# zafarrafii/Zaf-Python

Hardware: AMD Instinct MI355X
Metric: audio Msamples/sec (STFT win=2048 hop=1024) (higher is better)
Workload: dtype f32

## Files before the change

### zaf-python_amd/csrc/zafx_capi.cpp

```cpp
#include <dlfcn.h>

#include <algorithm>
#include <cmath>
#include <complex>
#include <cstdlib>
#include <cstring>
#include <map>
#include <mutex>
#include <string>
#include <utility>

#include "zafx_internal.hpp"

#ifndef ZAFX_STFT_FAT8_TABLES
#define ZAFX_STFT_FAT8_TABLES 0
#endif

namespace zafx {

static thread_local std::string g_err;
void set_error(const std::string& msg) { g_err = msg; }

hipError_t ensure_dynamic_lds(const void* kernel, int device, size_t bytes) {
    static std::mutex mu;
// ... 949 lines not shown
                    }
                    return cf32{(float)(scale * c), (float)(scale * sn)};
                };
                aux[(size_t)n] = root(2 * n * b2 + 2 * n * n, sin_);
                aux[(size_t)(N + n)] = root(2 * n * a2 + a2 * b2 + 2 * n * n + (sine ? 6 * D : 0), sout / L);
            }
            pl->kernel_name = "k_dct_bs32";
        } else {
            return bail("dct / dst: lengths above 8192 need N / 2 (types 2-4), N - 1 (dct type 1) or N + 1 (dst type 1) to be a power of two (at most 8192)");
        }
    } else {
        return bail("unknown plan kind");
    }
    pl->log2e = default_log2e(pl->log2nf);

    hipError_t e = hipSetDevice(device);
    if (e == hipSuccess) e = hipDeviceGetAttribute(&pl->n_cus, hipDeviceAttributeMultiprocessorCount, device);
    if (e == hipSuccess) e = hipStreamCreateWithFlags(&pl->stream, hipStreamNonBlocking);
    if (e == hipSuccess) e = hipEventCreate(&pl->ev0);
    if (e == hipSuccess) e = hipEventCreate(&pl->ev1);
    if (e == hipSuccess) {
        auto tw = is_cqt_family(kind) ? build_two_level_twiddles(pl->log2nf) : build_pass_twiddles(pl->log2nf, pl->log2e);
        if (is_cqt_family(kind) && cqt_split(pl->log2nf)) {
            const auto sub = build_pass_twiddles(10, 4);
            tw.insert(tw.end(), sub.begin(), sub.end());
        }
        if (tw.empty()) tw.push_back(cf32{1.f, 0.f});
        e = upload(&pl->d_tw_pass, tw.data(), tw.size() * sizeof(cf32));
        if (e == hipSuccess && (kind == ZAFX_STFT || kind == ZAFX_MEL || kind == ZAFX_MFCC) && (pl->log2nf == 10 || (ZAFX_STFT_FAT8_TABLES && pl->log2nf == 11 && kind == ZAFX_STFT))) {
            auto tw5 = build_pass_twiddles(pl->log2nf, 5);
            e = upload(&pl->d_tw_r32, tw5.data(), tw5.size() * sizeof(cf32));
        }
    }
    if (e == hipSuccess && (kind == ZAFX_STFT || kind == ZAFX_ISTFT || kind == ZAFX_MEL || kind == ZAFX_MFCC) && pl->log2nf == 11 && pl->prm.precision == ZAFX_PRECISION_F32) {
        const auto sub = build_pass_twiddles(10, 4);
        e = upload(&pl->d_tw_sub, sub.data(), sub.size() * sizeof(cf32));
    }
    if (e == hipSuccess && (kind == ZAFX_STFT || kind == ZAFX_ISTFT || kind == ZAFX_MEL || kind == ZAFX_MFCC) && pl->log2nf == 12 && pl->prm.precision == ZAFX_PRECISION_F32 && pl->bs_log2m == 0) {
        const auto sub = build_pass_twiddles(10, 4);
        e = upload(&pl->d_tw_sub, sub.data(), sub.size() * sizeof(cf32));
        std::vector<cf32> q(4096);
        for (int n = 0; n < 4096; ++n) q[(size_t)n] = unit_root(n, 8192);
        if (e == hipSuccess) e = upload(&pl->d_tw_quad, q.data(), q.size() * sizeof(cf32));
    }
    if (e == hipSuccess && kind == ZAFX_MDCT && pl->log2nf == 11 && pl->prm.precision == ZAFX_PRECISION_F32 && pl->bs_log2m == 0) {
        const auto sub = build_pass_twiddles(9, 3);
        e = upload(&pl->d_tw_sub, sub.data(), sub.size() * sizeof(cf32));
        std::vector<cf32> q(2048);
        for (int n = 0; n < 2048; ++n) q[(size_t)n] = unit_root(n, 2048);
        if (e == hipSuccess) e = upload(&pl->d_tw_quad, q.data(), q.size() * sizeof(cf32));
    }
    if (e == hipSuccess && kind == ZAFX_IMDCT && pl->log2nf == 11 && pl->prm.precision == ZAFX_PRECISION_F32 && pl->bs_log2m == 0) {
        const auto sub = build_pass_twiddles(10, 4);
        e = upload(&pl->d_tw_sub, sub.data(), sub.size() * sizeof(cf32));
        std::vector<cf32> q(2048);
        for (int n = 0; n < 2048; ++n) q[(size_t)n] = unit_root(n, 2048);
        if (e == hipSuccess) e = upload(&pl->d_tw_quad, q.data(), q.size() * sizeof(cf32));
    }
    if (e == hipSuccess && kind == ZAFX_MDCT && pl->log2nf == 10 && pl->prm.precision == ZAFX_PRECISION_F32 && pl->bs_log2m == 0) {
        const auto sub = build_pass_twiddles(9, 3);
        e = upload(&pl->d_tw_sub, sub.data(), sub.size() * sizeof(cf32));
        const int nf = pl->W / 4;
        std::vector<cf32> bt((size_t)nf + nf / 2);
        for (int s = 0; s < 2; ++s)
            for (int q = 0; q < nf / 2; ++q) bt[(size_t)s * (nf / 2) + q] = unit_root(8LL * (2 * q + s) + 1, 8LL * pl->W);
        for (int n = 0; n < nf / 2; ++n) bt[(size_t)nf + n] = unit_root(40LL * n + 1, 32LL * nf);
// ... 55 lines not shown
        } else if (cqt) {
            for (int k = 0; k < pl->W; ++k) tws[(size_t)k] = root(k, pl->W);
        } else {
            for (int k = 0; k <= n / 2; ++k) tws[(size_t)k] = root(k, pl->W);
        }
        if (e == hipSuccess) e = upload(&pl->d_tw64, tw.data(), tw.size() * sizeof(double2));
        if (e == hipSuccess) e = upload(&pl->d_tws64, tws.data(), tws.size() * sizeof(double2));
        pl->kernel_name = kind == ZAFX_STFT ? stft_f64_kernel_name() : kind == ZAFX_ISTFT ? istft_f64_kernel_name()
                          : kind == ZAFX_MDCT ? mdct_f64_kernel_name() : kind == ZAFX_IMDCT ? imdct_f64_kernel_name()
                          : cqt ? cqt_f64_kernel_name() : mel_f64_kernel_name();
        if (pl->bs_log2m > 0)
            pl->kernel_name = kind == ZAFX_ISTFT ? "k_ifft_frames_bs_f64" : kind == ZAFX_MDCT ? "k_mdct_bs_f64"
                              : kind == ZAFX_IMDCT ? "k_imdct_frames_bs_f64" : "k_stft_bs_f64";
    }
    if (e != hipSuccess) {
        zafx_plan_destroy(pl);
        return fail("zafx_plan_create", e);
    }
    *out = pl;
    return 0;
}

int zafx_plan_destroy(zafx_plan* pl) {
    if (!pl) return 0;
    (void)hipSetDevice(pl->device);
    if (pl->stream) (void)hipStreamSynchronize(pl->stream);
    for (int l = 0; l < 2; ++l)
        if (pl->lane_pcm[l]) (void)hipFree(pl->lane_pcm[l]);
    if (pl->d_window) (void)hipFree(pl->d_window);
    if (pl->d_matrix) (void)hipFree(pl->d_matrix);
    if (pl->d_wfold) (void)hipFree(pl->d_wfold);
    if (pl->d_tw_pass) (void)hipFree(pl->d_tw_pass);
    if (pl->d_tw_r32) (void)hipFree(pl->d_tw_r32);
    if (pl->d_tw_quad) (void)hipFree(pl->d_tw_quad);
    if (pl->d_tw_sub) (void)hipFree(pl->d_tw_sub);
    if (pl->d_tw_band) (void)hipFree(pl->d_tw_band);
    if (pl->d_fbw) (void)hipFree(pl->d_fbw);
    if (pl->d_fbw_meta) (void)hipFree(pl->d_fbw_meta);
    if (pl->d_dctw) (void)hipFree(pl->d_dctw);
    if (pl->d_tw_aux) (void)hipFree(pl->d_tw_aux);
    if (pl->d_indptr) (void)hipFree(pl->d_indptr);
    if (pl->d_indices) (void)hipFree(pl->d_indices);
    if (pl->d_values) (void)hipFree(pl->d_values);
    if (pl->d_cqt_waves) (void)hipFree(pl->d_cqt_waves);
    if (pl->d_cqt_addrs) (void)hipFree(pl->d_cqt_addrs);
    if (pl->d_cqt_vals) (void)hipFree(pl->d_cqt_vals);
    if (pl->d_cqt_mm_vals) (void)hipFree(pl->d_cqt_mm_vals);
    if (pl->d_cqt_mm_addr) (void)hipFree(pl->d_cqt_mm_addr);
    if (pl->d_cqt_mm_fin) (void)hipFree(pl->d_cqt_mm_fin);
    if (pl->d_window64) (void)hipFree(pl->d_window64);
    if (pl->d_tw64) (void)hipFree(pl->d_tw64);
    if (pl->d_tws64) (void)hipFree(pl->d_tws64);
    if (pl->d_scratch64) (void)hipFree(pl->d_scratch64);
    if (pl->d_fb64) (void)hipFree(pl->d_fb64);
    if (pl->d_fb64_meta) (void)hipFree(pl->d_fb64_meta);
    if (pl->d_dct64) (void)hipFree(pl->d_dct64);
    if (pl->d_cqt64_tw1) (void)hipFree(pl->d_cqt64_tw1);
    if (pl->d_cqt64_split) (void)hipFree(pl->d_cqt64_split);
    if (pl->d_cqt64_vals) (void)hipFree(pl->d_cqt64_vals);
    if (pl->d_cqt64_meta) (void)hipFree(pl->d_cqt64_meta);
    if (pl->d_cqt64_fin) (void)hipFree(pl->d_cqt64_fin);
    if (pl->d_mel64_stream) (void)hipFree(pl->d_mel64_stream);
    if (pl->d_mel64_fin) (void)hipFree(pl->d_mel64_fin);
    if (pl->d_mel64_dctT) (void)hipFree(pl->d_mel64_dctT);
    if (pl->d_values64) (void)hipFree(pl->d_values64);
    if (pl->d_bhat64) (void)hipFree(pl->d_bhat64);
// ... 838 lines not shown
```

### zaf-python_amd/csrc/zafx_fft.hpp

```cpp
#pragma once

#if defined(ZAFX_HOST_EMU)
#include <cmath>
struct float2 { float x, y; };
static inline float2 make_float2(float x, float y) { float2 r; r.x = x; r.y = y; return r; }
#define ZAFX_HD inline
#else
#include <hip/hip_runtime.h>

#include <type_traits>
#define ZAFX_HD __host__ __device__ __forceinline__
#endif

namespace zafx {

#if defined(__HIP_DEVICE_COMPILE__)
typedef float zafx_v2f __attribute__((ext_vector_type(2)));
__device__ __forceinline__ zafx_v2f to_v2(float2 a) { return __builtin_bit_cast(zafx_v2f, a); }
__device__ __forceinline__ float2 to_f2(zafx_v2f a) { return __builtin_bit_cast(float2, a); }
#define ZAFX_PK 1
#endif
#if defined(ZAFX_PK)
ZAFX_HD float2 cadd(float2 a, float2 b) { return to_f2(to_v2(a) + to_v2(b)); }
ZAFX_HD float2 csub(float2 a, float2 b) { return to_f2(to_v2(a) - to_v2(b)); }
// ... 339 lines not shown
#pragma unroll
            for (int r = 2; r < R; ++r) w[r] = cmul(w[r >> 1], w[r - (r >> 1)]);
#pragma unroll
            for (int r = 1; r < R; ++r) a[r] = cmul(a[r], w[r]);
        }
        Dft<R>::run(a);
        const int base = ((j >> LOG2NS) << (LOG2NS + LR)) + k;
        const int pb = phys_t<C::PS>(base);
#pragma unroll
        for (int r = 0; r < R; ++r) buf[phys_off<NS * R, C::PS>(pb, base, r * NS)] = a[r];
    }
}

#ifndef ZAFX_LDS_SINGLE
#define ZAFX_LDS_SINGLE 1
#endif
ZAFX_HD float2 lds_ld(const float2* p) {
#if ZAFX_LDS_SINGLE && defined(__HIP_DEVICE_COMPILE__)
    typedef __attribute__((address_space(3))) const volatile zafx_v2f lds_v2f;
    return to_f2(*(lds_v2f*)(p));
#else
    return *p;
#endif
}

template <int LOG2N, int LOG2E>
ZAFX_HD void regs_read(float2* v, const float2* buf, int p) {
    using C = FftCfg<LOG2N, LOG2E>;
    const int pp = phys_t<C::PS>(p);
#pragma unroll
    for (int i = 0; i < C::E; ++i) v[i] = buf[phys_off<C::P, C::PS>(pp, p, i * C::P)];
}

}

#if !defined(ZAFX_HOST_EMU) && defined(__HIPCC__)
namespace zafx {

__device__ __forceinline__ __amdgpu_buffer_rsrc_t make_rsrc(const void* base, unsigned bytes) {
    return __builtin_amdgcn_make_buffer_rsrc(const_cast<void*>(base), 0, (int)bytes, 0x00020000);
}
__device__ __forceinline__ float buf_load_f32(__amdgpu_buffer_rsrc_t r, int voff, int soff = 0) {
    return __builtin_bit_cast(float, __builtin_amdgcn_raw_buffer_load_b32(r, voff, soff, 0));
}
__device__ __forceinline__ int buf_load_i32(__amdgpu_buffer_rsrc_t r, int voff, int soff = 0) {
    return __builtin_bit_cast(int, __builtin_amdgcn_raw_buffer_load_b32(r, voff, soff, 0));
}
__device__ __forceinline__ float2 buf_load_f32x2(__amdgpu_buffer_rsrc_t r, int voff, int soff = 0) {
    const auto raw = __builtin_amdgcn_raw_buffer_load_b64(r, voff, soff, 0);
    float2 f;
    __builtin_memcpy(&f, &raw, 8);
    return f;
}

__device__ __forceinline__ float4 buf_load_f32x4(__amdgpu_buffer_rsrc_t r, int voff, int soff = 0) {
    const auto raw = __builtin_amdgcn_raw_buffer_load_b128(r, voff, soff, 0);
    float4 f;
    __builtin_memcpy(&f, &raw, 16);
    return f;
}

typedef float zafx_f32x2 __attribute__((ext_vector_type(2)));
__device__ __forceinline__ void store_stream(float2* p, float2 v) {
    zafx_f32x2 t;
    t.x = v.x;
    t.y = v.y;
// ... 235 lines not shown
```

### zaf-python_amd/csrc/zafx_internal.hpp

```cpp
#pragma once
#include <hip/hip_runtime.h>

#include <cstdint>
#include <atomic>
#include <string>
#include <type_traits>
#include <vector>

#include "../../include/zafx.h"
#include "zafx_twiddle.hpp"

namespace zafx {

constexpr int kMaxLdsBytes = 160 * 1024;
#ifndef ZAFX_CQT_SPLIT
#define ZAFX_CQT_SPLIT 1
#endif
constexpr bool cqt_double(int log2n) { return log2n == 15; }
constexpr int kCqtDoubleMaxBin = 8191;
constexpr bool cqt_split(int log2n) { return ZAFX_CQT_SPLIT && (log2n == 14 || log2n == 15); }
constexpr int kCqtRegion = 1090;
constexpr int cqt_slots(int log2n) { return cqt_split(log2n) ? 16 * kCqtRegion : (1 << log2n) + ((1 << log2n) >> 4) + 1; }
constexpr int cqt_slot14(int k) { return (k & 15) * kCqtRegion + (k >> 4) + (k >> 8); }
constexpr int cqt_slot(int log2n, int k) {
// ... 98 lines not shown
    int2* d_mel64_fin = nullptr;
    double* d_mel64_dctT = nullptr;
    int mel64_steps = 0, mel64_slots = 0, mel64_max_parts = 0, mel64_cpitch = 0, mel64_dct_half = 0;
    bool mel64_ok = false;
    double2* d_values64 = nullptr;
    double2* d_cqt64_tw1 = nullptr;
    int* d_cqt64_split = nullptr;
    double* d_cqt64_vals = nullptr;
    int* d_cqt64_meta = nullptr;
    int2* d_cqt64_fin = nullptr;
    int cqt64_kc2 = 0, cqt64_cols = 0, cqt64_steps = 0, cqt64_slots = 0, cqt64_max_parts = 0, cqt64_klo = 511;
    bool cqt64_ok = false, cqt64_dirty = true, cqt64_real = false;
    int bs_log2m = 0;
    void* d_pcm_float = nullptr;
    size_t pcm_float_bytes = 0;
    void* d_ragged = nullptr;
    size_t ragged_bytes = 0;
    void* h_ragged = nullptr;
    size_t ragged_host_bytes = 0;
    hipEvent_t rg_ev = nullptr;
    int dct_half = 0;
    long long dct_den2 = 0;
    float2* d_bs_chirp = nullptr;
    float2* d_bs_bhat = nullptr;
    double2* d_bhat64 = nullptr;
    std::vector<double2> h_values64;
    int cqt_k_lo = 0, cqt_k_hi = -1, cqt_k_special = 0;
    bool cqt_dirty = true;

    std::vector<float> h_window, h_fb, h_dct, h_matrix;
    std::vector<int32_t> h_indptr, h_indices;
    std::vector<zafx::cf32> h_values;

    std::string kernel_name;
    mutable std::atomic<const char*> ran{nullptr};
};

namespace zafx {

struct RgClip {
    long long in_off, n_samples, out_off;
    int T, TP, first_tile, pad_;
};
static_assert(sizeof(RgClip) == 40 && alignof(RgClip) == 8, "RgClip: the layout the host writes");
template <bool RAGGED>
using SamplesArg = std::conditional_t<RAGGED, const RgClip*, long long>;
template <bool RAGGED, class R, class A>
__host__ __device__ __forceinline__ const auto& rg_pick(const R& rec, const A& arg) {
    if constexpr (RAGGED) return rec;
    else return arg;
}
#ifdef __HIPCC__
__device__ __forceinline__ RgClip rg_clip(const RgClip* tab, int n_clips, int tl) {
    const int c = __builtin_amdgcn_readfirstlane(reinterpret_cast<const int*>(tab + n_clips)[tl]);
    return tab[c];
}
#endif
hipError_t launch_stft_ragged(const zafx_plan& pl, const float* x, float2* out, const RgClip* d_tab, int64_t n_clips, long long total_tiles, bool aligned);
hipError_t launch_mel_ragged(const zafx_plan& pl, const float* x, float* out, const RgClip* d_tab, int64_t n_clips, long long total_tiles, bool aligned);
bool spec2_ragged(const zafx_plan& pl);
bool stft_ragged_native(const zafx_plan& pl);
bool mel_ragged_native(const zafx_plan& pl);

inline int64_t row_pitch(const zafx_plan& pl, int64_t T) {
    const int64_t a = pl.prm.row_align;
    return (pl.layout == ZAFX_LAYOUT_FT && a > 1) ? (T + a - 1) / a * a : T;
}

hipError_t launch_stft(const zafx_plan& pl, const float* x, float2* out, int64_t n_clips, int64_t n_samples, int T);
hipError_t launch_istft(const zafx_plan& pl, const float2* spec, float* y, int64_t n_clips, int T, int64_t out_len);
hipError_t launch_stft_f64(const zafx_plan& pl, const double* x, double2* out, int64_t n_clips, int64_t n_samples, int T);
hipError_t launch_istft_f64(zafx_plan& pl, const double2* spec, double* y, int64_t n_clips, int T, int64_t out_len);
hipError_t launch_cqt_f64(zafx_plan& pl, const double* x, double* out, int64_t n_clips, int64_t n_samples, int T);
hipError_t launch_mel_f64(const zafx_plan& pl, const double* x, double* out, int64_t n_clips, int64_t n_samples, int T);
hipError_t launch_mdct_f64(const zafx_plan& pl, const double* x, double* out, int64_t n_clips, int64_t n_samples, int T);
hipError_t build_mel64_fb(zafx_plan& pl);
hipError_t build_mel64_dct(zafx_plan& pl);
hipError_t launch_imdct_f64(zafx_plan& pl, const double* coefs, double* y, int64_t n_clips, int T, int64_t out_len);
const char* stft_f64_kernel_name();
const char* istft_f64_kernel_name();
const char* mdct_f64_kernel_name();
const char* mel_f64_kernel_name();
const char* cqt_f64_kernel_name();
// ... 35 lines not shown

bool stft_supported(int log2n);
bool mdct_supported(int log2nf);
bool cqt_supported(int log2n);
int cqt_waves(int log2n);
int cqt_max_bins(int log2n);
int stft_frames_per_block(int log2n, int layout);
int mdct_frames_per_block(int log2nf, int layout);

void set_error(const std::string& msg);

int take_pcm_mode();
void set_pcm_mode(int mode);
bool pcm_mode_taken();

int carry_segments(long long n_clips, int tiles, long long grid);

hipError_t ensure_dynamic_lds(const void* kernel, int device, size_t bytes);

}

#ifdef ZAFX_PROF
#define ZAFX_PROF_ARRAY(name) __device__ unsigned long long name[16]; __device__ int name##_thread = 64;
#define PROF_INIT(name)                            \
    unsigned long long* const prof_ = name;        \
    const int prof_thread_ = name##_thread;        \
    unsigned long long tprev_ = __builtin_readcyclecounter()
#define PROF_MARK(i)                                                                       \
    do {                                                                                   \
        const unsigned long long now_ = __builtin_readcyclecounter();                     \
        if (blockIdx.x == 7 && (int)threadIdx.x == prof_thread_) atomicAdd(&prof_[i], now_ - tprev_);   \
        tprev_ = now_;                                                                     \
    } while (0)
#define ZAFX_PROF_EXPORT(fn, name)                                                                  \
    extern "C" int fn##_thread(int t) { return hipMemcpyToSymbol(HIP_SYMBOL(zafx::name##_thread), &t, sizeof(t)) != hipSuccess; } \
    extern "C" int fn(unsigned long long* out) {                                                    \
        unsigned long long zero[16] = {};                                                           \
        if (hipMemcpyFromSymbol(out, HIP_SYMBOL(zafx::name), sizeof(zero)) != hipSuccess) return 1; \
        return hipMemcpyToSymbol(HIP_SYMBOL(zafx::name), zero, sizeof(zero)) != hipSuccess;         \
    }
#else
#define ZAFX_PROF_ARRAY(name)
#define PROF_INIT(name)
#define PROF_MARK(i)
#define ZAFX_PROF_EXPORT(fn, name)
#endif
```

### zaf-python_amd/csrc/zafx_stft.hip

```cpp
#include <algorithm>
#include <type_traits>

#include "zafx_fft.hpp"
#include "zafx_internal.hpp"

namespace zafx {

template <int SPEC>
__device__ __forceinline__ float2* spec_base(float2* out, long long off) {
    if constexpr (SPEC >= 2) return reinterpret_cast<float2*>(reinterpret_cast<float*>(out) + off);
    else return out + off;
}
template <int SPEC, bool STREAM = false>
__device__ __forceinline__ void put_bin(float2* o, long long idx, float2 v) {
    if constexpr (SPEC >= 2) {
        const float pw = v.x * v.x + v.y * v.y;
        reinterpret_cast<float*>(o)[idx] = SPEC == 2 ? __builtin_amdgcn_sqrtf(pw) : pw;
    } else if constexpr (STREAM) {
        store_stream(o + idx, v);
    } else {
        o[idx] = v;
    }
}

// ... 77 lines not shown
                    put_bin<SPEC>(o, W - k, cconj(xk));
                    put_bin<SPEC>(o, N + k, cconj(xn));
                }
            }
        }
    } else {
        if constexpr (NT > 64) __syncthreads();
        const int tt = tid % FPB, kq = tid / FPB;
        if (t0 + tt >= T) return;
        const float2* fb = frames + tt * C::PITCH;
        float2* o = spec_base<SPEC>(out, (long long)clip * ROWS * TP + (t0 + tt));
        for (int k = kq; k < N / 2; k += P) {
            if (k == 0) {
                const float2 z0 = fb[0], zc = fb[phys(N / 2)];
                put_bin<SPEC>(o, 0, make_float2(z0.x + z0.y, 0.f));
                put_bin<SPEC>(o, (long long)N * TP, make_float2(z0.x - z0.y, 0.f));
                put_bin<SPEC>(o, (long long)(N / 2) * TP, cconj(zc));
                if (SPEC == 0) put_bin<SPEC>(o, (long long)(N + N / 2) * TP, zc);
            } else {
                float2 xk, xn;
                split_pair(fb[phys(k)], fb[phys(N - k)], tws[k], xk, xn);
                put_bin<SPEC>(o, (long long)k * TP, xk);
                put_bin<SPEC>(o, (long long)(N - k) * TP, xn);
                if (SPEC == 0) {
                    put_bin<SPEC>(o, (long long)(W - k) * TP, cconj(xk));
                    put_bin<SPEC>(o, (long long)(N + k) * TP, cconj(xn));
                }
            }
        }
    }
}

ZAFX_PROF_ARRAY(g_prof_stft)
constexpr int kFatWaves = 8;
constexpr int kFatFrames = 16;

template <int LOG2N, int LOG2E, int FPB_ = kFatFrames>
struct FatCfg {
    using C = FftCfg<LOG2N, LOG2E>;
    static_assert(C::P == 64 || C::P == 32, "a frame is owned by one wavefront, or by half of one (32 points per thread)");
    static constexpr int N = C::N;
    static constexpr int FPB = FPB_;
    static constexpr bool WIN_LDS = FPB_ == kFatFrames;
    static constexpr int PITCH = ((N + (N >> C::PS) + 31) / 32) * 32 + 32 / FPB_;
    static constexpr int NT = kFatWaves * 64;
    static constexpr int FPW = FPB_ * C::P / NT;
    static constexpr size_t SMEM = (size_t)(FPB_ * PITCH + C::TW + (WIN_LDS ? N : 0) + N / 2 + 1) * 8;
};

template <int PCM>
struct PcmPoint {
    using T = std::conditional_t<PCM == 1, float, float2>;
    static __device__ __forceinline__ float2 get(T v) {
        if constexpr (PCM == 1) {
            const int d = __builtin_bit_cast(int, v);
            return make_float2((float)(short)(d & 0xffff), (float)(d >> 16));
        } else if constexpr (PCM == 2) {
            const int a = __builtin_bit_cast(int, v.x), b = __builtin_bit_cast(int, v.y);
            return make_float2((float)((int)(short)(a & 0xffff) + (a >> 16)), (float)((int)(short)(b & 0xffff) + (b >> 16)));
        } else {
            return v;
        }
    }
    static constexpr float scale() { return PCM == 1 ? 1.f / 32768.f : PCM == 2 ? 1.f / 65536.f : 1.f; }
};

#ifndef ZAFX_STFT_FAT_OPAQUE
#define ZAFX_STFT_FAT_OPAQUE(log2n, spec) ((log2n) == 8 || ((log2n) == 9 && (spec) <= 1))
#endif
template <int LOG2N, int LOG2E, bool ALIGNED, int SPEC, int FPB_ = kFatFrames, int PCM = 0, bool RAGGED = false>
__global__ __launch_bounds__(kFatWaves * 64) void k_stft_ft16(
    const float* __restrict__ x, const float* __restrict__ win, const float2* __restrict__ twp,
    const float2* __restrict__ tws, float2* __restrict__ out, SamplesArg<RAGGED> n_samples, int hop, int T, int TP, int tiles,
    int total_tiles) {
    static_assert(!RAGGED || (PCM == 0 && FPB_ == kFatFrames), "ragged batches: float32 samples, 16-frame tiles");
#define CLIP_N rg_pick<RAGGED>(rc.n_samples, n_samples)
#define CLIP_T rg_pick<RAGGED>(rc.T, T)
#define CLIP_TP rg_pick<RAGGED>(rc.TP, TP)
    using C = FftCfg<LOG2N, LOG2E>;
    using F = FatCfg<LOG2N, LOG2E, FPB_>;
    constexpr int N = C::N, P = C::P, E = C::E, W = 2 * N, NT = F::NT, FPB = F::FPB, FPW = F::FPW, PITCH = F::PITCH;
    static_assert(FPW >= 1, "every group of P lanes transforms at least one frame per tile");
    constexpr int ROWS = SPEC ? N + 1 : W;
    extern __shared__ __attribute__((aligned(16))) unsigned char smem_raw[];
    float2* frames = reinterpret_cast<float2*>(smem_raw);
    float2* tw_l = frames + FPB * PITCH;
    float2* win_s = tw_l + C::TW;
    float2* tws_l = win_s + (F::WIN_LDS ? N : 0);
    const float2* win_l = F::WIN_LDS ? win_s : reinterpret_cast<const float2*>(win);
    const int tid = threadIdx.x;
    for (int i = tid; i < C::TW; i += NT) tw_l[i] = twp[i];
    static_assert(PCM == 0 || F::WIN_LDS, "int16 input: the staged window carries the scale");
    using PP = PcmPoint<PCM>;
    if constexpr (F::WIN_LDS)
        for (int i = tid; i < N; i += NT) {
            const float2 wv = reinterpret_cast<const float2*>(win)[i];
            win_s[i] = make_float2(wv.x * PP::scale(), wv.y * PP::scale());
        }
    for (int i = tid; i <= N / 2; i += NT) tws_l[i] = tws[i];
    __syncthreads();
    const int wave = tid / P, p_lane = tid % P, p = p_lane;
    const int tt = tid % FPB, kq = tid / FPB;
    const float2* fb = frames + tt * PITCH;
    const bool lines_whole = (RAGGED || TP % 16 == 0) && reinterpret_cast<uintptr_t>(out) % 128 == 0;

    typename PP::T xr[FPW][E];
    const bool xcd = ZAFX_XCD_ORDER && gridDim.x % 8 == 0;
    auto prefetch = [&](int tlv) {
        if (tlv >= total_tiles) return;
        const int tl = xcd ? xcd_order(tlv, total_tiles) : tlv;
        int p = p_lane;
        if constexpr (E >= 32 || ZAFX_STFT_FAT_OPAQUE(LOG2N, SPEC)) asm volatile("" : "+v"(p));
        [[maybe_unused]] RgClip rc;
        if constexpr (RAGGED) rc = rg_clip(n_samples, tiles, tl);
        const int clip = RAGGED ? 0 : tl / tiles, tile = RAGGED ? tl - rc.first_tile : tl % tiles;
        const float* xc = x + (RAGGED ? rc.in_off : (long long)clip * CLIP_N);
        const long long first = (long long)tile * FPB * hop - N;
        const long long last = first + (long long)(FPB - 1) * hop + W;
        if constexpr (PCM == 1) {
            const short* xs = reinterpret_cast<const short*>(x) + (long long)clip * CLIP_N;
            if (ALIGNED && first >= 0 && last <= CLIP_N && tile * FPB + FPB <= CLIP_T) {
                const short* src = xs + first + (long long)(wave * FPW) * hop + 2 * p;
#pragma unroll
                for (int f = 0; f < FPW; ++f) {
#pragma unroll
                    for (int i = 0; i < E; ++i) xr[f][i] = *reinterpret_cast<const float*>(src + (long long)f * hop + 2 * i * P);
                }
            } else {
#pragma unroll
                for (int f = 0; f < FPW; ++f) {
                    const int t = tile * FPB + wave * FPW + f;
                    const long long s0 = (long long)t * hop - N;
#pragma unroll
                    for (int i = 0; i < E; ++i) {
                        const long long s = s0 + 2 * (p + i * P);
                        const unsigned lo = (t < CLIP_T && s >= 0 && s < CLIP_N) ? (unsigned short)xs[s] : 0u;
                        const unsigned hi = (t < CLIP_T && s + 1 >= 0 && s + 1 < CLIP_N) ? (unsigned short)xs[s + 1] : 0u;
                        xr[f][i] = __builtin_bit_cast(float, lo | hi << 16);
                    }
                }
            }
        } else if (ALIGNED && first >= 0 && last <= CLIP_N && tile * FPB + FPB <= CLIP_T) {
            const float* src = xc + first + (long long)(wave * FPW) * hop + 2 * p;
#pragma unroll
            for (int f = 0; f < FPW; ++f) {
#pragma unroll
                for (int i = 0; i < E; ++i) xr[f][i] = *reinterpret_cast<const float2*>(src + (long long)f * hop + 2 * i * P);
            }
        } else {
#pragma unroll
            for (int f = 0; f < FPW; ++f) {
                const int t = tile * FPB + wave * FPW + f;
                const long long s0 = (long long)t * hop - N;
#pragma unroll
                for (int i = 0; i < E; ++i) {
                    const long long s = s0 + 2 * (p + i * P);
                    xr[f][i].x = (t < CLIP_T && s >= 0 && s < CLIP_N) ? xc[s] : 0.f;
                    xr[f][i].y = (t < CLIP_T && s + 1 >= 0 && s + 1 < CLIP_N) ? xc[s + 1] : 0.f;
                }
            }
        }
    };
    int tlv = blockIdx.x;
    prefetch(tlv);
    PROF_INIT(g_prof_stft);
    for (; tlv < total_tiles; tlv += gridDim.x) {
        const int tl = xcd ? xcd_order(tlv, total_tiles) : tlv;
        [[maybe_unused]] RgClip rc;
        if constexpr (RAGGED) rc = rg_clip(n_samples, tiles, tl);
        const int clip = RAGGED ? 0 : tl / tiles, tile = RAGGED ? tl - rc.first_tile : tl % tiles;
        const int t0 = tile * FPB;
        PROF_MARK(0);
        int po = p;
        if constexpr (E >= 32 || ZAFX_STFT_FAT_OPAQUE(LOG2N, SPEC)) asm volatile("" : "+v"(po));
#pragma unroll
        for (int f = 0; f < FPW; ++f) {
            float2 v[E];
#pragma unroll
            for (int i = 0; i < E; ++i) {
                const float2 wv = win_l[po + i * P], xv = PP::get(xr[f][i]);
                v[i] = make_float2(xv.x * wv.x, xv.y * wv.y);
            }
            fft_frame<LOG2N, LOG2E>(v, frames + (wave * FPW + f) * PITCH, po, tw_l);
        }
#ifndef ZAFX_STFT_EARLY
#define ZAFX_STFT_EARLY 1
#endif
        if (ZAFX_STFT_EARLY) prefetch(tlv + gridDim.x);
        PROF_MARK(1);
        lds_barrier();
        PROF_MARK(2);
        if (!ZAFX_STFT_EARLY) prefetch(tlv + gridDim.x);
        PROF_MARK(3);
        if (t0 + tt < CLIP_T) {
            float2* o = spec_base<SPEC>(out, (RAGGED ? rc.out_off : (long long)clip * ROWS * TP) + (t0 + tt));
            int kqo = kq;
            if constexpr (E >= 32 || ZAFX_STFT_FAT_OPAQUE(LOG2N, SPEC)) asm volatile("" : "+v"(kqo));
            auto store_tile = [&](auto stream) {
                constexpr bool ST = decltype(stream)::value;
                constexpr int ITER = (N / 2) / (NT / FPB);
#ifndef ZAFX_STFT_ROWROT_EXPR
#define ZAFX_STFT_ROWROT_EXPR (((int)blockIdx.x & 7) * 2 + ((int)blockIdx.x >> 3))
#endif
                static_assert((N / 2) % (NT / FPB) == 0, "the row sweep is a whole number of iterations");
                const int rot = ST ? ZAFX_STFT_ROWROT_EXPR : 0;
                for (int it = 0; it < ITER; ++it) {
                    const int k = kqo + ((it + rot) % ITER) * (NT / FPB);
                    if (k == 0) {
                        const float2 z0 = fb[0], zc = fb[phys_t<C::PS>(N / 2)];
                        put_bin<SPEC, ST>(o, 0, make_float2(z0.x + z0.y, 0.f));
                        put_bin<SPEC, ST>(o, (long long)N * CLIP_TP, make_float2(z0.x - z0.y, 0.f));
                        put_bin<SPEC, ST>(o, (long long)(N / 2) * CLIP_TP, cconj(zc));
                        if (SPEC == 0) put_bin<SPEC, ST>(o, (long long)(N + N / 2) * CLIP_TP, zc);
                    } else {
                        float2 xk, xn;
                        split_pair(fb[phys_t<C::PS>(k)], fb[phys_t<C::PS>(N - k)], tws_l[k], xk, xn);
                        put_bin<SPEC, ST>(o, (long long)k * CLIP_TP, xk);
                        if (SPEC == 0) put_bin<SPEC, ST>(o, (long long)(W - k) * CLIP_TP, cconj(xk));
                        put_bin<SPEC, ST>(o, (long long)(N - k) * CLIP_TP, xn);
                        if (SPEC == 0) put_bin<SPEC, ST>(o, (long long)(N + k) * CLIP_TP, cconj(xn));
                    }
                }
            };
#ifndef ZAFX_STFT_NO_NT
            if (SPEC < 2 && lines_whole && FPB == 16) store_tile(std::true_type{});
            else
#endif
                store_tile(std::false_type{});
        }
        PROF_MARK(4);
        lds_barrier();
    }
}
#undef CLIP_N
#undef CLIP_T
#undef CLIP_TP

template <int LOG2N, int LOG2E, bool ALIGNED, int SPEC, int PCM = 0>
__global__ __launch_bounds__(kFatWaves * 64) void k_stft_ft16c(
    const float* __restrict__ x, const float* __restrict__ win, const float2* __restrict__ twp,
    const float2* __restrict__ tws, float2* __restrict__ out, long long n_samples, int hop, int T, int TP, int tiles,
    int segs, int seg_tiles, int units) {
    static_assert(SPEC < 2, "complex spectra only (the real kinds write 64-byte runs)");
    using C = FftCfg<LOG2N, LOG2E>;
    using F = FatCfg<LOG2N, LOG2E>;
    constexpr int N = C::N, P = C::P, E = C::E, W = 2 * N, NT = F::NT, FPB = kFatFrames, FPW = F::FPW, PITCH = F::PITCH;
    constexpr int ROWS = SPEC ? N + 1 : W;
    constexpr int ITER = (N / 2) / (NT / FPB);
    static_assert((N / 2) % (NT / FPB) == 0 && ITER >= 1, "the row sweep is a whole number of iterations");
    extern __shared__ __attribute__((aligned(16))) unsigned char smem_raw[];
    float2* frames = reinterpret_cast<float2*>(smem_raw);
    float2* tw_l = frames + FPB * PITCH;
    float2* win_l = tw_l + C::TW;
    float2* tws_l = win_l + N;
    const int tid = threadIdx.x;
    for (int i = tid; i < C::TW; i += NT) tw_l[i] = twp[i];
    using PP = PcmPoint<PCM>;
    static_assert(PCM == 0 || ALIGNED, "int16 input: the buffer-load form");
    for (int i = tid; i < N; i += NT) {
        const float2 wv = reinterpret_cast<const float2*>(win)[i];
        win_l[i] = make_float2(wv.x * PP::scale(), wv.y * PP::scale());
    }
    for (int i = tid; i <= N / 2; i += NT) tws_l[i] = tws[i];
    __syncthreads();
// ... 1693 lines not shown
    if (f > cap) f = cap;
    if (f > lds_cap) f = lds_cap;
    int r = 1;
    while (r * 2 <= f) r *= 2;
    return r;
}

constexpr bool stft_use_fat(int log2n, int layout) {
    return layout == ZAFX_LAYOUT_FT && log2n >= 7 && log2n <= 10;
}

template <int LOG2N, bool ALIGNED, int SPEC>
static hipError_t run_stft_fat(const zafx_plan& pl, const float* x, float2* out, int64_t n_clips, int64_t n_samples, int T) {
#ifndef ZAFX_STFT_R32
#define ZAFX_STFT_R32 1
#endif
    constexpr int LOG2E = ((ZAFX_STFT_R32 && LOG2N == 10) || LOG2N == 11) ? 5 : default_log2e(LOG2N);
    constexpr int FPB = LOG2N == 11 ? 8 : kFatFrames;
    using F = FatCfg<LOG2N, LOG2E, FPB>;
    static_assert(F::SMEM <= (size_t)kMaxLdsBytes, "tile + tables exceed LDS");
    auto kern = k_stft_ft16<LOG2N, LOG2E, ALIGNED, SPEC, FPB>;
    if constexpr (LOG2N == 10 && SPEC < 2 && FPB == kFatFrames) {
        const int pcm = take_pcm_mode();
        if (pcm == 1) kern = k_stft_ft16<LOG2N, LOG2E, ALIGNED, SPEC, FPB, 1>;
        if (pcm == 2) kern = k_stft_ft16<LOG2N, LOG2E, ALIGNED, SPEC, FPB, 2>;
    }
    if (hipError_t e = ensure_dynamic_lds(reinterpret_cast<const void*>(kern), pl.device, F::SMEM); e != hipSuccess) return e;
    const int tiles = (T + FPB - 1) / FPB;
    const long long total = (long long)tiles * n_clips;
    if (total <= 0) return hipSuccess;
    const int per_cu = (int)std::min<size_t>(2, (size_t)kMaxLdsBytes / F::SMEM);
    const long long grid = std::min<long long>(total, (long long)pl.n_cus * std::max(per_cu, 1));
    pl.ran = "k_stft_ft16";
    hipLaunchKernelGGL(kern, dim3((unsigned)grid), dim3(F::NT), F::SMEM, pl.stream, x, pl.d_window, LOG2E == 5 ? pl.d_tw_r32 : pl.d_tw_pass,
                       pl.d_tw_aux, out, (long long)n_samples, pl.H, T, (int)row_pitch(pl, T), tiles, (int)total);
    return hipGetLastError();
}

template <int LOG2N, bool ALIGNED, int SPEC>
static hipError_t run_stft_fat_carry(const zafx_plan& pl, const float* x, float2* out, int64_t n_clips, int64_t n_samples, int T) {
    if constexpr (SPEC < 2) {
        constexpr int LOG2E = default_log2e(LOG2N);
        using F = FatCfg<LOG2N, LOG2E>;
        auto kern = k_stft_ft16c<LOG2N, LOG2E, ALIGNED, SPEC>;
        if constexpr (LOG2N == 10 && ALIGNED) {
            const int pcm = take_pcm_mode();
            if (pcm == 1) kern = k_stft_ft16c<LOG2N, LOG2E, true, SPEC, 1>;
            if (pcm == 2) kern = k_stft_ft16c<LOG2N, LOG2E, true, SPEC, 2>;
        }
        if (hipError_t e = ensure_dynamic_lds(reinterpret_cast<const void*>(kern), pl.device, F::SMEM); e != hipSuccess) return e;
        const int tiles = (T + kFatFrames - 1) / kFatFrames;
        if ((long long)tiles * n_clips <= 0) return hipSuccess;
        const long long max_grid = pl.n_cus;
        const int segs = carry_segments(n_clips, tiles, max_grid);
        const int seg_tiles = (tiles + segs - 1) / segs;
        const long long units = (long long)n_clips * segs;
        const long long grid = std::min<long long>(units, max_grid);
        pl.ran = "k_stft_ft16c";
        hipLaunchKernelGGL(kern, dim3((unsigned)grid), dim3(F::NT), F::SMEM, pl.stream, x, pl.d_window, pl.d_tw_pass, pl.d_tw_aux, out,
                           (long long)n_samples, pl.H, T, (int)row_pitch(pl, T), tiles, segs, seg_tiles, (int)units);
        return hipGetLastError();
    } else {
        return hipErrorInvalidValue;
    }
}

// ... 803 lines not shown
    const bool one = pl.prm.spectrum == ZAFX_SPECTRUM_ONE_SIDED;
    if (pl.layout == ZAFX_LAYOUT_FT)
        return one ? run_istft<L, ZAFX_LAYOUT_FT, true>(pl, spec, y, n_clips, T, out_len) : run_istft<L, ZAFX_LAYOUT_FT, false>(pl, spec, y, n_clips, T, out_len);
    return one ? run_istft<L, ZAFX_LAYOUT_TF, true>(pl, spec, y, n_clips, T, out_len) : run_istft<L, ZAFX_LAYOUT_TF, false>(pl, spec, y, n_clips, T, out_len);
}

hipError_t launch_stft(const zafx_plan& pl, const float* x, float2* out, int64_t n_clips, int64_t n_samples, int T) {
    if (hipError_t e = hipSuccess; launch_spec2(pl, x, reinterpret_cast<float*>(out), n_clips, n_samples, T, e)) return e;
    switch (pl.log2nf) {
#define X(L) \
    case L: return dispatch_stft<L>(pl, x, out, n_clips, n_samples, T);
        ZAFX_STFT_SIZES(X)
#undef X
    }
    return hipErrorInvalidValue;
}

bool stft_ragged_native(const zafx_plan& pl) {
    if (spec2_ragged(pl)) return true;
    return pl.kind == ZAFX_STFT && pl.prm.precision == ZAFX_PRECISION_F32 && pl.bs_log2m == 0 && pl.layout == ZAFX_LAYOUT_FT && pl.log2nf >= 7 &&
           pl.log2nf <= 10 && pl.d_tw_pass && pl.d_tw_aux && (pl.log2nf != 10 || !ZAFX_STFT_R32 || pl.d_tw_r32);
}

template <int LOG2N, bool ALIGNED, int SPEC>
static hipError_t run_stft_fat_ragged(const zafx_plan& pl, const float* x, float2* out, const RgClip* tab, int64_t n_clips, long long total_tiles) {
    constexpr int LOG2E = (ZAFX_STFT_R32 && LOG2N == 10) ? 5 : default_log2e(LOG2N);
    using F = FatCfg<LOG2N, LOG2E>;
    auto kern = k_stft_ft16<LOG2N, LOG2E, ALIGNED, SPEC, kFatFrames, 0, true>;
    if (hipError_t e = ensure_dynamic_lds(reinterpret_cast<const void*>(kern), pl.device, F::SMEM); e != hipSuccess) return e;
    if (total_tiles <= 0) return hipSuccess;
    const int per_cu = (int)std::min<size_t>(2, (size_t)kMaxLdsBytes / F::SMEM);
    const long long grid = std::min<long long>(total_tiles, (long long)pl.n_cus * std::max(per_cu, 1));
    pl.ran = "k_stft_ft16_ragged";
    hipLaunchKernelGGL(kern, dim3((unsigned)grid), dim3(F::NT), F::SMEM, pl.stream, x, pl.d_window, LOG2E == 5 ? pl.d_tw_r32 : pl.d_tw_pass,
                       pl.d_tw_aux, out, tab, pl.H, 0, 0, (int)n_clips, (int)total_tiles);
    return hipGetLastError();
}

template <int L>
static hipError_t dispatch_stft_ragged(const zafx_plan& pl, const float* x, float2* out, const RgClip* tab, int64_t n_clips, long long total_tiles, bool aligned) {
#define ZAFX_RAGGED_SPEC(S) \
    return aligned ? run_stft_fat_ragged<L, true, S>(pl, x, out, tab, n_clips, total_tiles) : run_stft_fat_ragged<L, false, S>(pl, x, out, tab, n_clips, total_tiles)
    switch (pl.prm.spectrum) {
        case ZAFX_SPECTRUM_ONE_SIDED: ZAFX_RAGGED_SPEC(1);
        case ZAFX_SPECTRUM_MAGNITUDE: ZAFX_RAGGED_SPEC(2);
        case ZAFX_SPECTRUM_POWER: ZAFX_RAGGED_SPEC(3);
        default: ZAFX_RAGGED_SPEC(0);
    }
#undef ZAFX_RAGGED_SPEC
}

hipError_t launch_stft_ragged(const zafx_plan& pl, const float* x, float2* out, const RgClip* tab, int64_t n_clips, long long total_tiles, bool aligned) {
    if (spec2_ragged(pl)) return launch_mel_ragged(pl, x, reinterpret_cast<float*>(out), tab, n_clips, total_tiles, aligned);
    switch (pl.log2nf) {
        case 7: return dispatch_stft_ragged<7>(pl, x, out, tab, n_clips, total_tiles, aligned);
        case 8: return dispatch_stft_ragged<8>(pl, x, out, tab, n_clips, total_tiles, aligned);
        case 9: return dispatch_stft_ragged<9>(pl, x, out, tab, n_clips, total_tiles, aligned);
        case 10: return dispatch_stft_ragged<10>(pl, x, out, tab, n_clips, total_tiles, aligned);
    }
    return hipErrorInvalidValue;
}

hipError_t launch_istft(const zafx_plan& pl, const float2* spec, float* y, int64_t n_clips, int T, int64_t out_len) {
    switch (pl.log2nf) {
#define X(L) \
    case L: return dispatch_istft<L>(pl, spec, y, n_clips, T, out_len);
        ZAFX_STFT_SIZES(X)
#undef X
    }
    return hipErrorInvalidValue;
}

}

ZAFX_PROF_EXPORT(zafx_debug_prof_istft, g_prof)
ZAFX_PROF_EXPORT(zafx_debug_prof_stft, g_prof_stft)
```

Baseline: 297,600.

## Claim STFT tiles dynamically via sharded atomic queues instead of static striding

Adds a dynamic tile scheduler to the fat STFT kernel. Blocks draw tiles from eight atomic counters keyed by block index and steal from neighbouring queues when their own is empty. The next tile is claimed during the last frame and staged in LDS double slots, so the prefetch still overlaps compute. The last block resets the counters for the next launch. The goal is to balance the tail across CUs, at the cost of global atomics per tile, a small extra LDS area, and dropping the XCD-aware ordering.

```diff
diff --git a/zaf-python_amd/csrc/zafx_capi.cpp b/zaf-python_amd/csrc/zafx_capi.cpp
--- a/zaf-python_amd/csrc/zafx_capi.cpp
+++ b/zaf-python_amd/csrc/zafx_capi.cpp
@@ -1005,6 +1005,12 @@
             e = upload(&pl->d_tw_r32, tw5.data(), tw5.size() * sizeof(cf32));
         }
     }
+    if (e == hipSuccess && kind == ZAFX_STFT && pl->prm.precision == ZAFX_PRECISION_F32) {
+        const std::vector<int> zeros((size_t)zafx::kClaimInts, 0);
+        e = upload(&pl->d_claim, zeros.data(), zeros.size() * sizeof(int));
+        const char* sw = std::getenv("ZAFX_STFT_DYNAMIC");
+        pl->stft_dynamic = !(sw && sw[0] == '0' && sw[1] == 0);
+    }
     if (e == hipSuccess && (kind == ZAFX_STFT || kind == ZAFX_ISTFT || kind == ZAFX_MEL || kind == ZAFX_MFCC) && pl->log2nf == 11 && pl->prm.precision == ZAFX_PRECISION_F32) {
         const auto sub = build_pass_twiddles(10, 4);
         e = upload(&pl->d_tw_sub, sub.data(), sub.size() * sizeof(cf32));
@@ -1126,6 +1132,8 @@
     if (pl->d_wfold) (void)hipFree(pl->d_wfold);
     if (pl->d_tw_pass) (void)hipFree(pl->d_tw_pass);
     if (pl->d_tw_r32) (void)hipFree(pl->d_tw_r32);
+    if (pl->d_claim) (void)hipFree(pl->d_claim);
+    if (pl->d_tail) (void)hipFree(pl->d_tail);
     if (pl->d_tw_quad) (void)hipFree(pl->d_tw_quad);
     if (pl->d_tw_sub) (void)hipFree(pl->d_tw_sub);
     if (pl->d_tw_band) (void)hipFree(pl->d_tw_band);
diff --git a/zaf-python_amd/csrc/zafx_fft.hpp b/zaf-python_amd/csrc/zafx_fft.hpp
--- a/zaf-python_amd/csrc/zafx_fft.hpp
+++ b/zaf-python_amd/csrc/zafx_fft.hpp
@@ -395,6 +395,25 @@
     for (int i = 0; i < C::E; ++i) v[i] = buf[phys_off<C::P, C::PS>(pp, p, i * C::P)];
 }
 
+constexpr int kClaimQueues = 8;
+constexpr int kClaimStride = 32;
+constexpr int kClaimInts = (kClaimQueues + 1) * kClaimStride;
+constexpr int kClaimLdsBytes = 16;
+ZAFX_HD int claim_len(int x, int total) { return (total >> 3) + (x < (total & 7) ? 1 : 0); }
+ZAFX_HD int claim_first(int x, int total) {
+    const int q = total >> 3, r = total & 7;
+    return x < r ? x * (q + 1) : r * (q + 1) + (x - r) * q;
+}
+template <class Draw>
+ZAFX_HD int claim_finish(int& q, int home, int total, int v, Draw draw) {
+    for (;;) {
+        if (v < claim_len(q, total)) return claim_first(q, total) + v;
+        q = (q + 1) & (kClaimQueues - 1);
+        if (q == home) return -1;
+        v = draw(q);
+    }
+}
+
 }
 
 #if !defined(ZAFX_HOST_EMU) && defined(__HIPCC__)
diff --git a/zaf-python_amd/csrc/zafx_internal.hpp b/zaf-python_amd/csrc/zafx_internal.hpp
--- a/zaf-python_amd/csrc/zafx_internal.hpp
+++ b/zaf-python_amd/csrc/zafx_internal.hpp
@@ -154,6 +154,9 @@
     std::vector<int32_t> h_indptr, h_indices;
     std::vector<zafx::cf32> h_values;
 
+    int* d_claim = nullptr;
+    bool stft_dynamic = false;
+    unsigned long long* d_tail = nullptr;
     std::string kernel_name;
     mutable std::atomic<const char*> ran{nullptr};
 };
@@ -171,6 +174,22 @@
 __host__ __device__ __forceinline__ const auto& rg_pick(const R& rec, const A& arg) {
     if constexpr (RAGGED) return rec;
     else return arg;
+}
+struct TileClaim {
+    int total_tiles, pad_;
+    int* counters;
+};
+template <bool DYN>
+using TilesArg = std::conditional_t<DYN, TileClaim, int>;
+template <bool DYN>
+__host__ __device__ __forceinline__ const int& tiles_total(const TilesArg<DYN>& a) {
+    if constexpr (DYN) return a.total_tiles;
+    else return a;
+}
+template <bool DYN>
+__host__ __device__ __forceinline__ int* tiles_claim(const TilesArg<DYN>& a) {
+    if constexpr (DYN) return a.counters;
+    else return nullptr;
 }
 #ifdef __HIPCC__
 __device__ __forceinline__ RgClip rg_clip(const RgClip* tab, int n_clips, int tl) {
@@ -272,6 +291,22 @@
         if (blockIdx.x == 7 && (int)threadIdx.x == prof_thread_) atomicAdd(&prof_[i], now_ - tprev_);   \
         tprev_ = now_;                                                                     \
     } while (0)
+#define ZAFX_PROF_TAIL_PTR(name) __device__ unsigned long long* name = nullptr;
+#define PROF_TAIL_INIT() \
+    const unsigned long long tail_t0_ = wall_clock64(); \
+    unsigned long long tail_first_ = 0, tail_n_ = 0
+#define PROF_TAIL_FIRST() do { if (tail_n_ == 0) tail_first_ = wall_clock64(); } while (0)
+#define PROF_TAIL_TILE() ++tail_n_
+#define PROF_TAIL_END(name)                                                     \
+    do {                                                                        \
+        unsigned long long* const tail_ = name;                                 \
+        if (tail_ && threadIdx.x == 0) {                                        \
+            tail_[4 * blockIdx.x + 0] = (blockIdx.x & 7) | tail_n_ << 8;        \
+            tail_[4 * blockIdx.x + 1] = tail_t0_;                               \
+            tail_[4 * blockIdx.x + 2] = tail_first_;                            \
+            tail_[4 * blockIdx.x + 3] = wall_clock64();                         \
+        }                                                                       \
+    } while (0)
 #define ZAFX_PROF_EXPORT(fn, name)                                                                  \
     extern "C" int fn##_thread(int t) { return hipMemcpyToSymbol(HIP_SYMBOL(zafx::name##_thread), &t, sizeof(t)) != hipSuccess; } \
     extern "C" int fn(unsigned long long* out) {                                                    \
@@ -283,5 +318,10 @@
 #define ZAFX_PROF_ARRAY(name)
 #define PROF_INIT(name)
 #define PROF_MARK(i)
+#define ZAFX_PROF_TAIL_PTR(name)
+#define PROF_TAIL_INIT()
+#define PROF_TAIL_FIRST()
+#define PROF_TAIL_TILE()
+#define PROF_TAIL_END(name)
 #define ZAFX_PROF_EXPORT(fn, name)
 #endif
diff --git a/zaf-python_amd/csrc/zafx_stft.hip b/zaf-python_amd/csrc/zafx_stft.hip
--- a/zaf-python_amd/csrc/zafx_stft.hip
+++ b/zaf-python_amd/csrc/zafx_stft.hip
@@ -133,6 +133,7 @@
 }
 
 ZAFX_PROF_ARRAY(g_prof_stft)
+ZAFX_PROF_TAIL_PTR(g_stft_tail)
 constexpr int kFatWaves = 8;
 constexpr int kFatFrames = 16;
 
@@ -169,12 +170,14 @@
 #ifndef ZAFX_STFT_FAT_OPAQUE
 #define ZAFX_STFT_FAT_OPAQUE(log2n, spec) ((log2n) == 8 || ((log2n) == 9 && (spec) <= 1))
 #endif
-template <int LOG2N, int LOG2E, bool ALIGNED, int SPEC, int FPB_ = kFatFrames, int PCM = 0, bool RAGGED = false>
+template <int LOG2N, int LOG2E, bool ALIGNED, int SPEC, int FPB_ = kFatFrames, int PCM = 0, bool RAGGED = false, bool DYN = false>
 __global__ __launch_bounds__(kFatWaves * 64) void k_stft_ft16(
     const float* __restrict__ x, const float* __restrict__ win, const float2* __restrict__ twp,
     const float2* __restrict__ tws, float2* __restrict__ out, SamplesArg<RAGGED> n_samples, int hop, int T, int TP, int tiles,
-    int total_tiles) {
+    TilesArg<DYN> tiles_arg) {
     static_assert(!RAGGED || (PCM == 0 && FPB_ == kFatFrames), "ragged batches: float32 samples, 16-frame tiles");
+    static_assert(!DYN || FPB_ == kFatFrames, "claimed tiles: 16-frame tiles");
+    const int& total_tiles = tiles_total<DYN>(tiles_arg);
 #define CLIP_N rg_pick<RAGGED>(rc.n_samples, n_samples)
 #define CLIP_T rg_pick<RAGGED>(rc.T, T)
 #define CLIP_TP rg_pick<RAGGED>(rc.TP, TP)
@@ -190,6 +193,20 @@
     float2* tws_l = win_s + (F::WIN_LDS ? N : 0);
     const float2* win_l = F::WIN_LDS ? win_s : reinterpret_cast<const float2*>(win);
     const int tid = threadIdx.x;
+    [[maybe_unused]] int* const slot = reinterpret_cast<int*>(tws_l + N / 2 + 1);
+    [[maybe_unused]] const int home = (int)blockIdx.x & (kClaimQueues - 1);
+    [[maybe_unused]] int cq = home, ticket = 0;
+    [[maybe_unused]] bool live = false;
+    [[maybe_unused]] auto draw = [&](int q) { return atomicAdd(tiles_claim<DYN>(tiles_arg) + q * kClaimStride, 1); };
+    if constexpr (DYN) {
+        if (tid == 0) {
+            const int c0 = claim_finish(cq, home, total_tiles, draw(cq), draw);
+            const int c1 = c0 >= 0 ? claim_finish(cq, home, total_tiles, draw(cq), draw) : -1;
+            slot[2] = c0;
+            slot[1] = c1;
+            live = c1 >= 0;
+        }
+    }
     for (int i = tid; i < C::TW; i += NT) tw_l[i] = twp[i];
     static_assert(PCM == 0 || F::WIN_LDS, "int16 input: the staged window carries the scale");
     using PP = PcmPoint<PCM>;
@@ -206,10 +223,10 @@
     const bool lines_whole = (RAGGED || TP % 16 == 0) && reinterpret_cast<uintptr_t>(out) % 128 == 0;
 
     typename PP::T xr[FPW][E];
-    const bool xcd = ZAFX_XCD_ORDER && gridDim.x % 8 == 0;
+    [[maybe_unused]] const bool xcd = ZAFX_XCD_ORDER && gridDim.x % 8 == 0;
     auto prefetch = [&](int tlv) {
-        if (tlv >= total_tiles) return;
-        const int tl = xcd ? xcd_order(tlv, total_tiles) : tlv;
+        if (DYN ? tlv < 0 : tlv >= total_tiles) return;
+        const int tl = DYN ? tlv : xcd ? xcd_order(tlv, total_tiles) : tlv;
         int p = p_lane;
         if constexpr (E >= 32 || ZAFX_STFT_FAT_OPAQUE(LOG2N, SPEC)) asm volatile("" : "+v"(p));
         [[maybe_unused]] RgClip rc;
@@ -263,10 +280,13 @@
         }
     };
     int tlv = blockIdx.x;
+    if constexpr (DYN) tlv = __builtin_amdgcn_readfirstlane(slot[2]);
+    [[maybe_unused]] int par = 0;
     prefetch(tlv);
     PROF_INIT(g_prof_stft);
-    for (; tlv < total_tiles; tlv += gridDim.x) {
-        const int tl = xcd ? xcd_order(tlv, total_tiles) : tlv;
+    PROF_TAIL_INIT();
+    while (DYN ? tlv >= 0 : tlv < total_tiles) {
+        const int tl = DYN ? tlv : xcd ? xcd_order(tlv, total_tiles) : tlv;
         [[maybe_unused]] RgClip rc;
         if constexpr (RAGGED) rc = rg_clip(n_samples, tiles, tl);
         const int clip = RAGGED ? 0 : tl / tiles, tile = RAGGED ? tl - rc.first_tile : tl % tiles;
@@ -277,6 +297,16 @@
 #pragma unroll
         for (int f = 0; f < FPW; ++f) {
             float2 v[E];
+            if constexpr (DYN) {
+                if (f == FPW - 1) {
+#pragma unroll
+                    for (int i = 0; i < E; ++i) {
+                        if constexpr (PCM == 1) asm volatile("" : "+v"(xr[f][i])::"memory");
+                        else asm volatile("" : "+v"(xr[f][i].x), "+v"(xr[f][i].y)::"memory");
+                    }
+                    if (tid == 0 && live) ticket = draw(cq);
+                }
+            }
 #pragma unroll
             for (int i = 0; i < E; ++i) {
                 const float2 wv = win_l[po + i * P], xv = PP::get(xr[f][i]);
@@ -287,11 +317,21 @@
 #ifndef ZAFX_STFT_EARLY
 #define ZAFX_STFT_EARLY 1
 #endif
-        if (ZAFX_STFT_EARLY) prefetch(tlv + gridDim.x);
+        if constexpr (DYN) {
+            if (tid == 0) {
+                const int c = live ? claim_finish(cq, home, total_tiles, ticket, draw) : -1;
+                slot[par] = c;
+                live = c >= 0;
+            }
+        }
+        int nxt = tlv + gridDim.x;
+        if constexpr (DYN) nxt = __builtin_amdgcn_readfirstlane(slot[par ^ 1]);
+        if (ZAFX_STFT_EARLY) prefetch(nxt);
         PROF_MARK(1);
         lds_barrier();
         PROF_MARK(2);
-        if (!ZAFX_STFT_EARLY) prefetch(tlv + gridDim.x);
+        if (!ZAFX_STFT_EARLY) prefetch(nxt);
+        PROF_TAIL_FIRST();
         PROF_MARK(3);
         if (t0 + tt < CLIP_T) {
             float2* o = spec_base<SPEC>(out, (RAGGED ? rc.out_off : (long long)clip * ROWS * TP) + (t0 + tt));
@@ -331,6 +371,17 @@
         }
         PROF_MARK(4);
         lds_barrier();
+        tlv = nxt;
+        par ^= 1;
+        PROF_TAIL_TILE();
+    }
+    PROF_TAIL_END(g_stft_tail);
+    if constexpr (DYN) {
+        if (tid == 0) {
+            int* const cnt = tiles_claim<DYN>(tiles_arg);
+            if (atomicAdd(cnt + kClaimQueues * kClaimStride, 1) == (int)gridDim.x - 1)
+                for (int i = 0; i <= kClaimQueues; ++i) atomicExch(cnt + i * kClaimStride, 0);
+        }
     }
 }
 #undef CLIP_N
@@ -2090,6 +2141,18 @@
     const int per_cu = (int)std::min<size_t>(2, (size_t)kMaxLdsBytes / F::SMEM);
     const long long grid = std::min<long long>(total, (long long)pl.n_cus * std::max(per_cu, 1));
     pl.ran = "k_stft_ft16";
+    if constexpr (SPEC < 2 && FPB == kFatFrames) {
+        if (pl.stft_dynamic && pl.d_claim && kern == k_stft_ft16<LOG2N, LOG2E, ALIGNED, SPEC, FPB> && row_pitch(pl, T) % 16 == 0 &&
+            reinterpret_cast<uintptr_t>(out) % 128 == 0) {
+            static_assert(F::SMEM + kClaimLdsBytes <= (size_t)kMaxLdsBytes, "tile + tables + claim words exceed LDS");
+            auto dyn = k_stft_ft16<LOG2N, LOG2E, ALIGNED, SPEC, FPB, 0, false, true>;
+            if (hipError_t e = ensure_dynamic_lds(reinterpret_cast<const void*>(dyn), pl.device, F::SMEM + kClaimLdsBytes); e != hipSuccess) return e;
+            hipLaunchKernelGGL(dyn, dim3((unsigned)grid), dim3(F::NT), F::SMEM + kClaimLdsBytes, pl.stream, x, pl.d_window,
+                               LOG2E == 5 ? pl.d_tw_r32 : pl.d_tw_pass, pl.d_tw_aux, out, (long long)n_samples, pl.H, T, (int)row_pitch(pl, T), tiles,
+                               TileClaim{(int)total, 0, pl.d_claim});
+            return hipGetLastError();
+        }
+    }
     hipLaunchKernelGGL(kern, dim3((unsigned)grid), dim3(F::NT), F::SMEM, pl.stream, x, pl.d_window, LOG2E == 5 ? pl.d_tw_r32 : pl.d_tw_pass,
                        pl.d_tw_aux, out, (long long)n_samples, pl.H, T, (int)row_pitch(pl, T), tiles, (int)total);
     return hipGetLastError();
@@ -2959,6 +3022,14 @@
     const int per_cu = (int)std::min<size_t>(2, (size_t)kMaxLdsBytes / F::SMEM);
     const long long grid = std::min<long long>(total_tiles, (long long)pl.n_cus * std::max(per_cu, 1));
     pl.ran = "k_stft_ft16_ragged";
+    if (pl.stft_dynamic && pl.d_claim) {
+        static_assert(F::SMEM + kClaimLdsBytes <= (size_t)kMaxLdsBytes, "tile + tables + claim words exceed LDS");
+        auto dyn = k_stft_ft16<LOG2N, LOG2E, ALIGNED, SPEC, kFatFrames, 0, true, true>;
+        if (hipError_t e = ensure_dynamic_lds(reinterpret_cast<const void*>(dyn), pl.device, F::SMEM + kClaimLdsBytes); e != hipSuccess) return e;
+        hipLaunchKernelGGL(dyn, dim3((unsigned)grid), dim3(F::NT), F::SMEM + kClaimLdsBytes, pl.stream, x, pl.d_window,
+                           LOG2E == 5 ? pl.d_tw_r32 : pl.d_tw_pass, pl.d_tw_aux, out, tab, pl.H, 0, 0, (int)n_clips, TileClaim{(int)total_tiles, 0, pl.d_claim});
+        return hipGetLastError();
+    }
     hipLaunchKernelGGL(kern, dim3((unsigned)grid), dim3(F::NT), F::SMEM, pl.stream, x, pl.d_window, LOG2E == 5 ? pl.d_tw_r32 : pl.d_tw_pass,
                        pl.d_tw_aux, out, tab, pl.H, 0, 0, (int)n_clips, (int)total_tiles);
     return hipGetLastError();
@@ -3002,3 +3073,19 @@
 
 ZAFX_PROF_EXPORT(zafx_debug_prof_istft, g_prof)
 ZAFX_PROF_EXPORT(zafx_debug_prof_stft, g_prof_stft)
+#ifdef ZAFX_PROF
+extern "C" int zafx_debug_stft_tail_bind(zafx_plan* pl, int on) {
+    if (!pl || hipSetDevice(pl->device) != hipSuccess) return 1;
+    const size_t bytes = (size_t)pl->n_cus * 2 * 4 * sizeof(unsigned long long);
+    if (on && !pl->d_tail && hipMalloc(reinterpret_cast<void**>(&pl->d_tail), bytes) != hipSuccess) return 1;
+    if (hipStreamSynchronize(pl->stream) != hipSuccess) return 1;
+    if (on && hipMemset(pl->d_tail, 0, bytes) != hipSuccess) return 1;
+    unsigned long long* p = on ? pl->d_tail : nullptr;
+    return hipMemcpyToSymbol(HIP_SYMBOL(zafx::g_stft_tail), &p, sizeof(p)) != hipSuccess;
+}
+extern "C" int zafx_debug_stft_tail_read(zafx_plan* pl, unsigned long long* out, int n_words) {
+    if (!pl || !pl->d_tail || n_words > pl->n_cus * 2 * 4) return 1;
+    if (hipStreamSynchronize(pl->stream) != hipSuccess) return 1;
+    return hipMemcpy(out, pl->d_tail, (size_t)n_words * sizeof(unsigned long long), hipMemcpyDeviceToHost) != hipSuccess;
+}
+#endif
```

Result: faster. 302,200, median of 6 (+1.6%).
